# blackfeather-wang/AdaFocus

Measured on AMD Instinct MI355X. Metric: clips/sec (T=16, patch=96^2, ResNet-50 local), higher is better.
Workload: dtype f32; 1 GPU; ActivityNet AdaFocus hot path: gather + ResNet-50 local CNN + GRU classifier, T=16, P=96, B=64 clips/GPU (1024 patches/GPU/step), random-init weights seed 1007; global_batch=64, frames=16, patch=96, parallelism=dp1, streams=3

## Files before the change

### adafocus_amd/csrc/adaf_internal.h

```cpp
#pragma once
#include <hip/hip_runtime.h>
#include <stdint.h>
#include <stddef.h>
#include <string>

#include "../../include/adafocus.h"
#include <type_traits>

struct adaf_handle {
    int device = 0;
    int cus = 256;
    float* zeros = nullptr;
    unsigned* scan_timeouts = nullptr;
    int conv_pos_major = 1;
    int gru_persistent = 1;
    hipEvent_t scan_done[4] = {nullptr, nullptr, nullptr, nullptr};
    bool scan_used[4] = {false, false, false, false};
    int scan_next = 0;
    int scan_resident = 0;
    int scan_slots = 1;
    int bptt_resident = 0;
    std::string err;
};

#include <mutex>
#include <vector>
struct AdafAuxPool {
    struct Aux { hipStream_t key = nullptr; hipStream_t stream = nullptr; hipEvent_t ev_fork = nullptr, ev_join = nullptr; unsigned long long used = 0; };
    static constexpr size_t kMax = 16;
    std::vector<Aux> entries;
    std::mutex mu;
    unsigned long long tick = 0;
    AdafAuxPool() { entries.reserve(kMax); }
    bool create(Aux* a) {
        return hipStreamCreateWithFlags(&a->stream, hipStreamNonBlocking) == hipSuccess &&
               hipEventCreateWithFlags(&a->ev_fork, hipEventDisableTiming) == hipSuccess &&
               hipEventCreateWithFlags(&a->ev_join, hipEventDisableTiming) == hipSuccess;
    }
    void prepare(size_t count) {
        std::lock_guard<std::mutex> lk(mu);
        while (entries.size() < count && entries.size() < kMax) {
            Aux a;
            if (!create(&a)) return;
            entries.push_back(a);
        }
    }
// ... 51 lines not shown
    explicit AdafCarver(void* ws) : base(static_cast<char*>(ws)) {}
    template <typename T> T* take(size_t count, size_t align = sizeof(T)) {
        T* p = base ? reinterpret_cast<T*>(base + off) : nullptr;
        off += (count * sizeof(T) + align - 1) / align * align;
        return p;
    }
};

struct AdafOptions {
    int conv_pool = 1;
    int mb_strip = 1;
    int mbv2_chunk = 512;
    int latency_rows = 1536;
    int latency_linear_rows = 128;
    unsigned effnet_plan = 511u;
    unsigned effnet_fused_blocks = 0xffffffffu;
    int effnet_chunk = 1024;
    int stem_rows = 1;
    int split_stage1_f32 = 1;
    int split_lean = 1;
    int tsm_lean = 1;
    int gru_graph_persistent = 0;
    int gru_scan_slices = 2;
};
AdafOptions& adaf_options();

__device__ __forceinline__ _Float16 adaf_f16_of(float v) {
#if defined(__HIP_DEVICE_COMPILE__)
    asm("" : "+v"(v));
#endif
    return (_Float16)v;
}

struct ConvArgs {
    const float* x;
    const float* w;
    const unsigned short* wsp;
    const float* scale;
    const float* bias;
    const float* res;
    float* out;
    int M, N, K;
    int cin, H, W, OH, OW, KH, KW, stride, pad;
    int ldx, ldo, ldr;
    int act;
    int tsm_T, tsm_fold, tsm_hw;
// ... 122 lines not shown
bool adaf_gru_scan_persistent_ok(int batch, int hidden, int classes, int resident_blocks);
int adaf_gru_scan_groups(int batch, int resident_blocks);
struct AdafGruScanPlan {
    int groups;
    int bpad;
    size_t nzero;
};
AdafGruScanPlan adaf_gru_scan_plan(int batch, int steps, size_t bar_words, int resident_blocks);
hipError_t adaf_launch_gru_scan_persistent(const float* gi, const float* whh, const float* bhh, const float* h0, float* hs,
                                           unsigned* bar, const AdafGruScanPlan& plan, int batch, int steps, const float* fcw, const float* fcb,
                                           float* logits, float* last, int classes, bool cooperative, unsigned* timeouts, hipStream_t s);

int adaf_gru_bptt_blocks_per_cu();
bool adaf_gru_bptt_persistent_ok(int batch, int hidden, int resident_blocks);
hipError_t adaf_launch_gru_bptt(const float* dy, const float* gi, const float* gh, const float* bhh, const float* hs, const float* whh,
                                float* dgi, float* dgh, float* carry, unsigned* bar, unsigned* timeouts, int batch, int steps, int hidden,
                                bool persistent, bool cooperative, hipStream_t s);
void adaf_launch_gemm_strided(const float* A, long long a_m, long long a_k, const float* B, long long b_k, long long b_n, float* C, int ldc,
                              const float* mul, int ldm, int M, int N, int K, hipStream_t s);
size_t adaf_colsum_partial_floats(int cols);
void adaf_launch_colsum(const float* x, int rows, int cols, int ld, float* part, float* out, hipStream_t s);
void adaf_launch_rows_scale(const float* x, const float* mask, float* out, int rows, int width, int steps, bool shift, hipStream_t s);

int adaf_launch_conv_gemm(const ConvArgs& a, int tile, int cus, hipStream_t s);
int adaf_pick_conv_tile(int M, int N, int K, int cus);
int adaf_launch_conv_lat(const ConvArgs& a, hipStream_t s);
int adaf_launch_conv_pool(ConvArgs a, int hw, float* pool_out, int pool_ld, hipStream_t s);
int adaf_launch_conv_pool16(ConvArgs a, int hw, float* pool_out, int pool_ld, hipStream_t s);
int adaf_launch_conv_pool16_rounded(ConvArgs a, int hw, float* pool_out, int pool_ld, hipStream_t s);
bool adaf_conv_tile_exists(int tile);
void adaf_launch_conv_naive(const ConvArgs& a, hipStream_t s);
bool adaf_fused_tail_shift_ok(const ConvArgs& c2, int n3, int ldr, int tsm_T1, int tsm_fold1);
int adaf_launch_fused_tail(const ConvArgs& c2, const float* w3, const float* s3, const float* b3, const float* res, int ldr,
                           float* out, int n3, const float* w1n, const float* s1n, const float* b1n, float* out1, int n1,
                           hipStream_t s, int tsm_T1 = 0, int tsm_fold1 = 0);

hipError_t adaf_launch_crop(const float* frames, int nf, int C, int H, int W, const float* act, int fpa, int P,
                            float* out, int layout, int32_t* coords, hipStream_t s);

hipError_t adaf_launch_crop_resize(const float* frames, int in4, int nf, int C, int H, int W, const float* act, const int32_t* sizes,
                                   int size_default, int fpa, int P, float* out, int layout, int32_t* coords, hipStream_t s);
hipError_t adaf_launch_resize_nearest(const float* frames, int in4, int nf, int C, int H, int W, int OH, int OW, float* out,
                                      int layout, hipStream_t s);

void adaf_launch_split_weight(const float* w, size_t count, unsigned short* planes, hipStream_t s);
void adaf_launch_pack_weight(const float* w, int cout, int cin, int kh, int kw, int cin_pad, float* o, hipStream_t s);
void adaf_launch_fold_bn(const float* g, const float* b, const float* m, const float* v, float eps, int c,
                         float* scale, float* bias, hipStream_t s);
// ... 36 lines not shown
```

### adafocus_amd/csrc/api.hip

```cpp
#include <cstdarg>
#include <cstdio>
#include <cstring>

#include "adaf_internal.h"

int adaf_fail(adaf_handle* h, int code, const char* fmt, ...) {
    char buf[512];
    va_list ap;
    va_start(ap, fmt);
    vsnprintf(buf, sizeof(buf), fmt, ap);
    va_end(ap);
    if (h) h->err = buf;
    return code;
}

int adaf_hip_fail(adaf_handle* h, hipError_t e, const char* what) {
    return adaf_fail(h, ADAF_E_LAUNCH, "%s: %s", what, hipGetErrorString(e));
}

bool adaf_aligned16(const void* p) { return (reinterpret_cast<uintptr_t>(p) & 15) == 0; }
int adaf_check_ws(adaf_handle* h, const char* who, const void* ws, size_t ws_bytes, size_t need, AdafWsOrder order) {
    const bool small = ws_bytes < need, skew = !adaf_aligned16(ws);
    if (small && (order == ADAF_WS_SIZE_FIRST || !skew)) return adaf_fail(h, ADAF_E_NOMEM, "%s: workspace %zu < %zu bytes", who, ws_bytes, need);
    return skew ? adaf_fail(h, ADAF_E_LAYOUT, "%s: the workspace must be 16-byte aligned", who) : ADAF_OK;
// ... 37 lines not shown
    a->vec_epi = (p->cout % 4 == 0 && ldo % 4 == 0 && ldr % 4 == 0 && adaf_aligned16(out) && (!res || adaf_aligned16(res)) &&
                  (!scale || adaf_aligned16(scale)) && (!bias || adaf_aligned16(bias))) ? 1 : 0;
    return ADAF_OK;
}

int adaf_set_conv_dtypes(adaf_handle* h, bool in16, bool out16, ConvArgs* a) {
    a->in16 = in16; a->out16 = out16; a->res16 = a->res != nullptr;
    if (in16 && (a->cin % 8 || a->ldx % 8)) return adaf_fail(h, ADAF_E_LAYOUT, "conv_f16: fp16 operands need cin %% 8 == 0 (16-byte chunks)");
    if (in16 && a->tsm_T > 0 && a->tsm_fold % 8)
        return adaf_fail(h, ADAF_E_LAYOUT, "conv_f16: temporal-shift fold=%d must be a multiple of 8 with fp16 operands (whole 16-byte chunks)", a->tsm_fold);
    if (!in16 && a->res) return adaf_fail(h, ADAF_E_BADARG, "conv_f16: a residual needs fp16 operands");
    return ADAF_OK;
}

AdafOptions& adaf_options() {
    static AdafOptions o;
    return o;
}

namespace {
struct OptKey { const char* name; double lo, hi; };
const OptKey kOptKeys[] = {{"conv_pool", 0, 1}, {"mb_strip", 0, 1}, {"mbv2_chunk", 1, 1 << 20}, {"latency_rows", 0, 1 << 30}, {"latency_linear_rows", 0, 1 << 30},
                           {"effnet_plan", 0, 511}, {"effnet_chunk", 1, 1 << 20}, {"gru_scan_slices", 1, 2}, {"effnet_fused_blocks", 0, 4294967295.0},
                           {"stem_rows", 0, 2}, {"split_stage1_f32", 0, 1}, {"gru_graph_persistent", 0, 1}, {"split_lean", 0, 1}, {"tsm_lean", 0, 1}};
int find_opt(const char* key) {
    if (!key) return -1;
    for (size_t i = 0; i < sizeof(kOptKeys) / sizeof(kOptKeys[0]); ++i)
        if (!strcmp(kOptKeys[i].name, key)) return (int)i;
    return -1;
}
}

extern "C" {

int adaf_version(void) { return ADAF_VERSION; }

int adaf_create(int device, adaf_handle** out) {
    if (!out) return ADAF_E_BADARG;
    *out = nullptr;
    int count = 0;
    if (hipGetDeviceCount(&count) != hipSuccess || device < 0 || device >= count) return ADAF_E_ARCH;
    hipDeviceProp_t prop;
    if (hipGetDeviceProperties(&prop, device) != hipSuccess) return ADAF_E_ARCH;
    if (strncmp(prop.gcnArchName, "gfx950", 6) != 0) return ADAF_E_ARCH;
    adaf_handle* h = new adaf_handle();
    h->device = device;
    h->cus = prop.multiProcessorCount > 0 ? prop.multiProcessorCount : 256;
// ... 5 lines not shown
    if (e == hipSuccess) e = hipMalloc(reinterpret_cast<void**>(&h->scan_timeouts), 256);
    if (e == hipSuccess) e = hipMemset(h->scan_timeouts, 0, 256);
    for (int i = 0; i < 4 && e == hipSuccess; ++i) e = hipEventCreateWithFlags(&h->scan_done[i], hipEventDisableTiming);
    if (e == hipSuccess) {
        const int per_cu = adaf_gru_scan_blocks_per_cu();
        h->scan_resident = (per_cu > 1 ? per_cu - 1 : per_cu) * h->cus;
        const int slots = h->scan_resident / 128;
        h->scan_slots = slots < 1 ? 1 : (slots > 4 ? 4 : slots);
        const int bptt_per_cu = adaf_gru_bptt_blocks_per_cu();
        h->bptt_resident = (bptt_per_cu > 1 ? bptt_per_cu - 1 : bptt_per_cu) * h->cus;
    }
    (void)hipSetDevice(cur);
    if (e != hipSuccess) { delete h; return ADAF_E_NOMEM; }
    *out = h;
    return ADAF_OK;
}

int adaf_destroy(adaf_handle* h) {
    if (h && h->zeros) (void)hipFree(h->zeros);
    if (h && h->scan_timeouts) (void)hipFree(h->scan_timeouts);
    if (h)
        for (int i = 0; i < 4; ++i)
            if (h->scan_done[i]) (void)hipEventDestroy(h->scan_done[i]);
    delete h;
    return ADAF_OK;
}

const char* adaf_last_error(const adaf_handle* h) { return h ? h->err.c_str() : "null handle"; }
int adaf_device_cus(const adaf_handle* h) { return h ? h->cus : 0; }
int adaf_set_conv_pos_major(adaf_handle* h, int on) {
    if (!h) return ADAF_E_BADARG;
    h->conv_pos_major = on < 0 || on > 2 ? 1 : on;
    return ADAF_OK;
}
int adaf_set_global_option(const char* key, double value) {
    const int k = find_opt(key);
    if (k < 0 || !(value >= kOptKeys[k].lo && value <= kOptKeys[k].hi)) return ADAF_E_BADARG;
    AdafOptions& o = adaf_options();
    switch (k) {
        case 0: o.conv_pool = (int)value; break;
        case 1: o.mb_strip = (int)value; break;
        case 2: o.mbv2_chunk = (int)value; break;
        case 3: o.latency_rows = (int)value; break;
        case 4: o.latency_linear_rows = (int)value; break;
        case 5: o.effnet_plan = (unsigned)value; break;
        case 6: o.effnet_chunk = (int)value; break;
        case 7: o.gru_scan_slices = (int)value; break;
        case 8: o.effnet_fused_blocks = (unsigned)value; break;
        case 9: o.stem_rows = (int)value; break;
        case 10: o.split_stage1_f32 = (int)value; break;
        case 11: o.gru_graph_persistent = (int)value; break;
        case 12: o.split_lean = (int)value; break;
        default: o.tsm_lean = (int)value; break;
    }
    return ADAF_OK;
}

double adaf_get_global_option(const char* key) {
    const AdafOptions& o = adaf_options();
    switch (find_opt(key)) {
        case 0: return o.conv_pool;
        case 1: return o.mb_strip;
        case 2: return o.mbv2_chunk;
        case 3: return o.latency_rows;
        case 4: return o.latency_linear_rows;
        case 5: return o.effnet_plan;
        case 6: return o.effnet_chunk;
        case 7: return o.gru_scan_slices;
        case 8: return o.effnet_fused_blocks;
        case 9: return o.stem_rows;
        case 10: return o.split_stage1_f32;
        case 11: return o.gru_graph_persistent;
        case 12: return o.split_lean;
        case 13: return o.tsm_lean;
        default: return __builtin_nan("");
    }
}

int adaf_set_gru_persistent(adaf_handle* h, int on) {
    if (!h) return ADAF_E_BADARG;
    if (on < 0 || on > 2) return adaf_fail(h, ADAF_E_BADARG, "set_gru_persistent: mode %d (0 off, 1 on, 2 on + cooperative launch)", on);
    h->gru_persistent = on;
    return ADAF_OK;
}

int adaf_gru_scan_timeouts(adaf_handle* h, unsigned* count_out) {
    if (!h || !count_out) return ADAF_E_BADARG;
    int cur = 0;
    (void)hipGetDevice(&cur);
    (void)hipSetDevice(h->device);
    hipError_t e = hipDeviceSynchronize();
    if (e == hipSuccess) e = hipMemcpy(count_out, h->scan_timeouts, sizeof(unsigned), hipMemcpyDeviceToHost);
    (void)hipSetDevice(cur);
    return e == hipSuccess ? ADAF_OK : adaf_hip_fail(h, e, "gru_scan_timeouts");
}

int adaf_crop_gather_f32(adaf_handle* h, const float* frames, int n_frames, int channels, int height, int width,
// ... 520 lines not shown
```

### adafocus_amd/csrc/conv_gemm.hip

```cpp
#include <cstdlib>
#include <type_traits>
#include <utility>

#include "adaf_internal.h"

typedef float f32x16 __attribute__((ext_vector_type(16)));
typedef float f32x4 __attribute__((ext_vector_type(4)));
typedef float f32x2 __attribute__((ext_vector_type(2)));
typedef unsigned u32x4 __attribute__((ext_vector_type(4)));
typedef __bf16 bf16x8 __attribute__((ext_vector_type(8)));
typedef _Float16 f16x8 __attribute__((ext_vector_type(8)));
typedef _Float16 f16x4 __attribute__((ext_vector_type(4)));

#ifndef CG_ABL
#define CG_ABL 0
#endif

namespace {

typedef __bf16 bf16x2 __attribute__((ext_vector_type(2)));
__device__ __forceinline__ void split3(const f32x4 v0, const f32x4 v1, u32x4& H, u32x4& M, u32x4& L) {
    const float x[8] = {v0.x, v0.y, v0.z, v0.w, v1.x, v1.y, v1.z, v1.w};
    unsigned h[4], m[4], l[4];
#pragma unroll
// ... 1447 lines not shown
    else if (a.act == ADAF_ACT_SWISH) v = v / (1.f + expf(-v));
    a.out[(size_t)m * a.ldo + n] = v;
}

enum TileFamily {
    TF_REG,
    TF_DMA_TOP,
    TF_DMA_MID,
    TF_BAR23,
    TF_SPLIT6,
    TF_SPLIT9,
    TF_PRESPLIT,
    TF_F16,
    TF_LAT,
};
struct TileRow {
    int id;
    int bm, bn;
    int wgm, wgn;
    TileFamily fam;
    int fallback;
    int presplit;
    float eff;
};
constexpr int kTileAutoSplit = 40;
constexpr TileRow kTileTable[] = {
    {1, 128, 128, 2, 2, TF_REG, 0, 0, 1.00f},
    {2, 128, 64, 2, 2, TF_REG, 0, 0, 1.02f},
    {3, 64, 64, 2, 2, TF_REG, 0, 0, 0.98f},
    {4, 64, 128, 2, 2, TF_REG, 0, 0, 0.99f},
    {5, 256, 128, 4, 2, TF_REG, 0, 0, 0.f},
    {21, 128, 128, 2, 2, TF_DMA_TOP, 1, 0, 0.f},
    {22, 128, 64, 2, 2, TF_DMA_TOP, 2, 0, 0.f},
    {23, 64, 64, 2, 2, TF_DMA_TOP, 3, 0, 0.f},
    {24, 64, 128, 2, 2, TF_DMA_TOP, 4, 0, 0.f},
    {25, 256, 128, 4, 2, TF_DMA_TOP, 5, 0, 0.f},
    {26, 256, 128, 2, 2, TF_DMA_TOP, 1, 0, 0.f},
    {31, 128, 128, 2, 2, TF_DMA_MID, 1, 0, 0.f},
    {32, 128, 64, 2, 2, TF_DMA_MID, 2, 0, 0.f},
    {33, 64, 64, 2, 2, TF_DMA_MID, 3, 0, 0.f},
    {34, 64, 128, 2, 2, TF_DMA_MID, 4, 0, 0.f},
    {38, 128, 32, 4, 1, TF_DMA_MID, 1, 0, 0.f},
    {39, 256, 32, 4, 1, TF_DMA_MID, 1, 0, 0.f},
    {41, 128, 128, 2, 2, TF_SPLIT6, 1, 65, 0.f},
    {42, 128, 64, 2, 2, TF_SPLIT6, 2, 62, 0.f},
    {43, 64, 64, 2, 2, TF_SPLIT6, 3, 63, 0.f},
    {44, 64, 128, 2, 2, TF_SPLIT6, 4, 64, 0.f},
    {45, 256, 128, 4, 2, TF_SPLIT6, 5, 0, 0.f},
    {46, 256, 128, 2, 2, TF_SPLIT6, 1, 0, 0.f},
    {51, 128, 128, 2, 2, TF_SPLIT9, 1, 0, 0.f},
    {52, 128, 64, 2, 2, TF_SPLIT9, 2, 0, 0.f},
    {53, 64, 64, 2, 2, TF_SPLIT9, 3, 0, 0.f},
    {54, 64, 128, 2, 2, TF_SPLIT9, 4, 0, 0.f},
// ... 63 lines not shown
};

bool conv_is_dense(const ConvArgs& a) { return a.KH == 1 && a.KW == 1 && a.stride == 1 && a.pad == 0; }
int conv_images(const ConvArgs& a) { return a.OH * a.OW > 0 ? a.M / (a.OH * a.OW) : 0; }

bool dma_reach(size_t elems, size_t elem_bytes = 4) { return elems * elem_bytes < 0xffffff00ull; }
bool operands_in_dma_reach(const ConvArgs& a) {
    return dma_reach((size_t)a.M * a.ldx) && dma_reach((size_t)a.N * a.K) &&
           (conv_is_dense(a) || dma_reach((size_t)a.H * a.W * a.ldx * (size_t)conv_images(a)));
}
bool strided_1x1_as_gather(const ConvArgs& a) {
    return !conv_is_dense(a) && a.KH == 1 && a.KW == 1 && a.pad == 0 && a.stride > 1 && a.tsm_T == 0 && (a.K & 31) == 0;
}

double conv_tap_fill(const ConvArgs& a) {
    auto axis = [&](int out, int in, int k) {
        long long c = 0;
        for (int o = 0; o < out; ++o)
            for (int t = 0; t < k; ++t) c += (unsigned)(o * a.stride - a.pad + t) < (unsigned)in;
        return c;
    };
    return (double)(axis(a.OH, a.H, a.KH) * axis(a.OW, a.W, a.KW)) / ((double)a.OH * a.OW * a.KH * a.KW);
}
bool pos_major_gate(const ConvArgs& a, const TileRow& r) {
    const int ohw = a.OH * a.OW, images = conv_images(a);
    return has_pos_major_form(r) && (r.fam == TF_PRESPLIT ? a.pm_allow == 1 : a.pm_allow != 0) && !conv_is_dense(a) && a.KH * a.KW > 1 &&
           a.KH * a.KW <= 32 && images * ohw == a.M && images >= r.bm && ohw <= 4096 && conv_tap_fill(a) < 0.96;
}
bool lean_shift_gate(const ConvArgs& a, const TileRow& r) {
    return has_lean_shift_form(r) && conv_is_dense(a) && a.tsm_T > 0 && (a.K & 31) == 0 && (a.tsm_fold & 31) == 0 && a.stride == 1 &&
           operands_in_dma_reach(a) && adaf_options().tsm_lean && (size_t)a.M * a.ldx * 4 < 0x7fff0000ull;
}

bool adaf_conv_glds_ok(const ConvArgs& a) {
    if (conv_is_dense(a)) return a.K % 4 == 0;
    return a.K % 32 == 0 && a.cin % 32 == 0 && a.KH * a.KW <= 32;
}

bool conv_glds16_ok(const ConvArgs& a) {
    if ((a.K & 1) || (a.cin & 1) || (a.ldx & 1)) return false;
    if (conv_is_dense(a)) return (a.K / 2) % 4 == 0;
    return (a.K / 2) % 32 == 0 && (a.cin / 2) % 32 == 0 && a.KH * a.KW <= 32;
}

bool narrow_output(const ConvArgs& a) { return (((a.N + 63) / 64) * 64 - a.N) * 5 >= a.N; }
long long row_tiles(const ConvArgs& a, int bm) { return (a.M + bm - 1) / bm; }

int resolve_f32_tile(const ConvArgs& a, int tile, int cus) {
    const bool dma_ok = adaf_conv_glds_ok(a);
    const bool presplit_ok = a.wsp != nullptr && (a.K & 31) == 0 && dma_ok;
    if (tile == kTileAutoSplit) {
        tile = 0;
        if (dma_ok) {
            if (a.N <= 64) tile = family_tile(TF_SPLIT6, 128, 64);
            else if (row_tiles(a, 128) * ((a.N + 127) / 128) * 2 >= cus) tile = family_tile(TF_SPLIT6, 128, 128);
            else tile = family_tile_like(TF_SPLIT6, adaf_pick_conv_tile(a.M, a.N, a.K, cus));
            if (presplit_ok) tile = kTileTable[tile_index(tile)].presplit;
        }
    }
    if (tile <= 0) {
        tile = adaf_pick_conv_tile(a.M, a.N, a.K, cus);
        if (dma_ok) {
            tile = family_tile_like(TF_DMA_MID, tile);
            if (narrow_output(a) && row_tiles(a, 128) >= cus) tile = family_tile(TF_DMA_MID, 128, 32);
            else if (narrow_output(a) && a.K >= 512 && row_tiles(a, 256) * ((a.N + 31) / 32) >= cus) tile = family_tile(TF_DMA_MID, 256, 32);
        }
    }
    for (int i = tile_index(tile); i >= 0; i = tile_index(tile)) {
        const TileRow& r = kTileTable[i];
        if (r.fam == TF_REG || (r.fam == TF_PRESPLIT ? presplit_ok : dma_ok && r.fam != TF_F16 && r.fam != TF_LAT)) return tile;
        tile = r.fallback;
    }
    return -1;
}

void plan_row_major(ConvPlan& p, const ConvArgs& a, int tile, int bm_rows) {
    p.row = tile_index(p.tile = tile);
    p.a.tiles_n = (a.N + kTileTable[p.row].bn - 1) / kTileTable[p.row].bn;
    p.a.nblocks = ((a.M + bm_rows - 1) / bm_rows) * p.a.tiles_n;
}

ConvPlan plan_conv(const ConvArgs& a, int tile, int cus) {
    ConvPlan p(a);
    const bool dense = conv_is_dense(a);
    if (a.in16) {
        if (!conv_glds16_ok(a) || (a.res && !a.res16)) return p;
        if (tile < kTileF16Lo || tile > kTileF16Hi) {
            tile = family_tile_like(TF_F16, adaf_pick_conv_tile(a.M, a.N, a.K, cus));
            if (narrow_output(a) && row_tiles(a, 128) >= cus) tile = family_tile(TF_F16, 128, 32);
        }
        if (tile_index(tile) < 0) return p;
        plan_row_major(p, a, tile, kTileTable[tile_index(tile)].bm);
        p.a.K /= 2; p.a.cin /= 2; p.a.ldx /= 2; p.a.tsm_fold /= 2;
        p.dt = DT_IN16 | DT_RES16 | (a.out16 ? DT_OUT16 : 0);
        p.dense = dense;
        p.special = dense && (a.tsm_T > 0 || (p.a.K & 31));
        return p;
    }
    if (a.out16) {
        if (a.res) return p;
        plan_row_major(p, a, kTileOut16, kTileTable[tile_index(kTileOut16)].bm);
        p.dt = DT_OUT16;
        p.dense = dense;
        return p;
    }
    const int asked = tile_index(tile);
    if (asked >= 0 && kTileTable[asked].fam == TF_LAT) {
        p.row = tile_index(p.tile = tile);
        return p;
    }
    tile = resolve_f32_tile(a, tile, cus);
    if (tile < 0) return p;
    const TileRow& r = kTileTable[tile_index(tile)];
    plan_row_major(p, a, tile, r.bm);
    if (a.vec_epi) p.a.vec_epi = 2;
    p.dense = dense;
    if (r.fam == TF_REG) return p;
    const bool special = a.tsm_T > 0 || (a.K & 31);
    p.special = dense && special;
    const bool lean = has_lean_form(r) && operands_in_dma_reach(a) &&
                      (r.fam != TF_PRESPLIT || (adaf_options().split_lean && dma_reach((size_t)3 * a.N * a.K, 2)));
    if (pos_major_gate(a, r)) {
        p.pos_major = true;
        p.lean = lean && a.pm_allow != 2;
        p.a.pm_images = conv_images(a);
        p.a.pm_groups = (p.a.pm_images + r.bm - 1) / r.bm;
        p.a.nblocks = a.OH * a.OW * p.a.pm_groups * p.a.tiles_n;
    } else if ((dense || strided_1x1_as_gather(a)) && !special && lean && lean_dense_pays(r)) {
        p.gather = !dense;
        p.dense = p.lean = true;
    } else if (lean_shift_gate(a, r)) {
        p.lean = true;
    }
    return p;
// ... 70 lines not shown
}

template <int... I>
int launch_rows(const ConvPlan& p, const ConvArgs& a, hipStream_t s, std::integer_sequence<int, I...>) {
    int rc = -1;
    (void)((p.row == I && ((rc = launch_row<I>(p, a, s)), true)) || ...);
    return rc;
}

int launch_plan(const ConvPlan& p, hipStream_t s) {
    return p.tile < 0 ? -1 : launch_rows(p, p.a, s, std::make_integer_sequence<int, kNumTiles>());
}

int launch_conv_pool(const ConvArgs& a, int hw, float* pool_out, int pool_ld, PoolKind kind, hipStream_t s) {
    ConvPlan p = plan_conv_pool(a, hw, pool_out, pool_ld, kind);
    if (p.tile < 0) return 0;
    p.a.pool_hw = hw; p.a.pool_rows = (128 / hw) * hw; p.a.pool_out = pool_out; p.a.pool_ld = pool_ld;
    launch_plan(p, s);
    return 1;
}

}

int adaf_pick_conv_tile(int M, int N, int K, int cus) {
    (void)K;
    int best = 1;
    double best_t = 1e300;
    for (const TileRow& r : kTileTable) {
        if (r.eff <= 0.f) continue;
        const long long blocks = (long long)((M + r.bm - 1) / r.bm) * ((N + r.bn - 1) / r.bn);
        const long long rounds = (blocks + cus - 1) / cus;
        const double cost = (double)rounds * r.bm * r.bn / r.eff;
        if (cost < best_t * 0.999) { best_t = cost; best = r.id; }
    }
    return best;
}

bool adaf_conv_tile_exists(int tile) { return tile == kTileAutoSplit || tile_index(tile) >= 0; }

int adaf_launch_conv_gemm(const ConvArgs& a, int tile, int cus, hipStream_t s) { return launch_plan(plan_conv(a, tile, cus), s); }

int adaf_launch_conv_pool(ConvArgs a, int hw, float* pool_out, int pool_ld, hipStream_t s) {
    return launch_conv_pool(a, hw, pool_out, pool_ld, POOL_F32, s);
}

int adaf_launch_conv_pool16(ConvArgs a, int hw, float* pool_out, int pool_ld, hipStream_t s) {
    return launch_conv_pool(a, hw, pool_out, pool_ld, POOL_F16, s);
}

int adaf_launch_conv_pool16_rounded(ConvArgs a, int hw, float* pool_out, int pool_ld, hipStream_t s) {
    return launch_conv_pool(a, hw, pool_out, pool_ld, POOL_F16_ROUNDED, s);
}

extern "C" int adaf_conv_plan_debug(const adaf_conv_params* p, int flags, int cus, int* out, int n) {
    enum { IN16 = 1, OUT16 = 2, RES16 = 4, PRESPLIT = 8, VEC_EPI = 64 };
    alignas(16) static const float operand[4] = {0.f, 0.f, 0.f, 0.f};
    alignas(16) static float result[4];
    if (!out || cus <= 0) return ADAF_E_BADARG;
    adaf_handle host;
    ConvArgs a;
    int rc = adaf_make_conv_args(&host, p, operand, operand, nullptr, nullptr, (flags & RES16) ? operand : nullptr, result, &a);
    if (!rc && (flags & (IN16 | OUT16 | RES16))) rc = adaf_set_conv_dtypes(&host, (flags & IN16) != 0, (flags & OUT16) != 0, &a);
    if (rc) return rc;
    if (flags & PRESPLIT) a.wsp = reinterpret_cast<const unsigned short*>(operand);
    a.pm_allow = (flags >> 4) & 3;
    a.vec_epi = a.vec_epi && (flags & VEC_EPI);
    const int hw = flags >> 8;
    const ConvPlan c = hw > 0 ? plan_conv_pool(a, hw, operand, p->cout, !a.in16 ? POOL_F32 : a.res16 ? POOL_F16_ROUNDED : POOL_F16)
                              : plan_conv(a, p->tile, cus);
    const TileRow r = c.row >= 0 ? kTileTable[c.row] : TileRow{0, 0, 0, 0, 0, TF_REG, 0, 0, 0.f};
    const int kPlanFields[] = {c.tile, r.bm, r.bn, r.wgm, r.wgn, (int)r.fam, r.fallback, family_pipe(r.fam), family_split(r.fam),
                               r.fam == TF_PRESPLIT, c.dt, c.dense, c.gather, c.special, c.lean, c.pos_major, c.pool, c.a.tiles_n, c.a.nblocks,
                               c.a.pm_images, c.a.pm_groups, c.a.vec_epi, c.a.K, c.a.cin, c.a.ldx, c.a.tsm_fold};
    for (int i = 0; i < n && i < (int)(sizeof(kPlanFields) / sizeof(int)); ++i) out[i] = kPlanFields[i];
    return ADAF_OK;
}

void adaf_launch_conv_naive(const ConvArgs& a, hipStream_t s) {
    const long long total = (long long)a.M * a.N;
    hipLaunchKernelGGL(conv_naive_kernel, dim3((unsigned)((total + 255) / 256)), dim3(256), 0, s, a);
}

static bool fused_tail_pm(const ConvArgs& c2, int n3, int ldr, int* images_out, int* groups_out, int gstride = 128) {
    const int ohw = c2.OH * c2.OW;
    const int images = ohw > 0 ? c2.M / ohw : 0;
    const int groups = (images + gstride - 1) / gstride;
    *images_out = images;
    *groups_out = groups;
    return c2.pm_allow == 1 && images * ohw == c2.M && images >= 128 && ohw <= 4096 &&
           (long long)groups * 128 * 100 <= (long long)images * (gstride == 128 ? 106 : 108) && (size_t)ohw * 8 * (size_t)(n3 > ldr ? n3 : ldr) * 4 < 0xffffff00ull;
}

static int fused_tail_gstride(int tsm_T1) { return tsm_T1 > 0 && tsm_T1 <= 128 ? (128 / tsm_T1) * tsm_T1 : 128; }
// ... 48 lines not shown
```

### adafocus_amd/csrc/resnet_trunk.hip

```cpp
#include <cstdio>
#include <cstring>
#include <string>
#include <vector>

#include "adaf_net.h"

struct ConvLayer : AdafNetConv {
    int pad;
    bool tsm = false;
    unsigned short* wsp = nullptr;
};

struct adaf_resnet50 {
    adaf_handle* h = nullptr;
    AdafParamTable params;
    AdafWeightArena arena;
    std::vector<ConvLayer> convs;
    std::vector<int> tiles;
    int blocks[4] = {3, 4, 6, 3};
    float* l10_w = nullptr;
    float* l10_scale = nullptr;
    float* l10_bias = nullptr;
    unsigned short* l10_w16 = nullptr;
    int math = ADAF_MATH_F32;
// ... 48 lines not shown
    int nframes, H, W;
    const float* act;
    int fpa;
};

adaf_conv_params layer_params(const ConvLayer& L, int n, int hh, int ww, int act) {
    adaf_conv_params p;
    memset(&p, 0, sizeof(p));
    p.n = n; p.h = hh; p.w = ww; p.cin = L.cin_pad; p.cout = L.cout; p.kh = p.kw = L.k; p.stride = L.stride; p.pad = L.pad;
    p.act = act;
    return p;
}

size_t trunk_layout(const adaf_resnet50* net, int n, int patch, void* ws, float* buf[6]) {
    const int s1 = adaf_conv_out(patch, 7, 2, 3), s2 = adaf_conv_out(s1, 3, 2, 1);
    const size_t a = (size_t)s1 * s1 * 64, b = (size_t)s2 * s2 * 256;
    AdafCarver c(ws);
    for (int i = 0; i < 6; ++i) buf[i] = (i < 5 || (net && net->tsm_block)) ? c.take<float>((a > b ? a : b) * n) : nullptr;
    return c.off;
}

inline const float* as_f32(const void* p) { return static_cast<const float*>(p); }

int run_trunk(adaf_resnet50* net, const float* x4, int n, int P, int tsm_T, int tsm_div, float* feat, int ldfeat,
              void* ws, size_t ws_bytes, hipStream_t st, std::vector<hipEvent_t>* rec, std::vector<Launch>* info, float* featmap = nullptr,
              const FrameSrc* src = nullptr) {
    adaf_handle* h = net->h;
    if (src) x4 = src->frames;
    if (!net->finalized) return adaf_fail(h, ADAF_E_STATE, "resnet50: finalize() has not been called");
    if (!x4 || !feat || !ws) return adaf_fail(h, ADAF_E_BADARG, "resnet50: null pointer");
    if (n <= 0 || P < 32) return adaf_fail(h, ADAF_E_BADARG, "resnet50: need n > 0 and patch >= 32");
    if (ldfeat == 0) ldfeat = 2048;
    if (ldfeat < 2048 || ldfeat % 4 || !adaf_aligned16(feat) || !adaf_aligned16(x4) || !adaf_aligned16(ws))
        return adaf_fail(h, ADAF_E_LAYOUT, "resnet50: ldfeat >= 2048, %% 4 == 0 and 16-byte aligned buffers required");
    if (tsm_T > 0 && n % tsm_T) return adaf_fail(h, ADAF_E_BADARG, "resnet50: n=%d not a multiple of tsm_segments=%d", n, tsm_T);
    float* buf[6];
    if (int rc = adaf_check_ws(h, "resnet50", ws, ws_bytes, trunk_layout(net, n, P, ws, buf), ADAF_WS_ALIGN_FIRST)) return rc;

    const int lat_rows = net->lat_rows >= 0 ? net->lat_rows : adaf_options().latency_rows;
    const bool lat_ok = lat_rows > 0 && tsm_T == 0 && net->math == ADAF_MATH_F32;
    const bool fuse = net->fuse;
    const bool stage1_f32 = net->math == ADAF_MATH_F32 || (net->math == ADAF_MATH_F32_SPLIT_BF16 && adaf_options().split_stage1_f32);
    const bool tsm_block = net->tsm_block && tsm_T > 0;
    const int tsm_c1 = tsm_block ? 0 : tsm_T;

    const bool f16 = net->math == ADAF_MATH_F16;
    const double eb = f16 ? 2.0 : 4.0;
    const char* tag = f16 ? " (fp16)" : "";
    if (f16) {
        if (!net->convs[1].w16) return adaf_fail(h, ADAF_E_STATE, "resnet50: fp16 filters missing (finalize() did not complete)");
        if (tsm_T > 0 && tsm_div <= 0) return adaf_fail(h, ADAF_E_BADARG, "resnet50: tsm_div must be positive");
        if (tsm_c1 > 0)
            for (size_t i = 1; i < net->convs.size(); ++i) {
                const ConvLayer& L = net->convs[i];
                if (L.tsm && (L.cin / tsm_div) % 8)
                    return adaf_fail(h, ADAF_E_LAYOUT, "resnet50 (fp16): temporal-shift fold = %d / %d = %d of %s must be a multiple of 8", L.cin, tsm_div,
                                     L.cin / tsm_div, L.name.c_str());
            }
    }
    auto bank = [&](const ConvLayer& L) { return f16 ? as_f32(L.w16) : L.w; };
    const float* const l10_w = f16 ? as_f32(net->l10_w16) : (stage1_f32 ? net->l10_w : nullptr);

    auto mark = [&](double flops, double bytes, int tile) {
        if (rec) {
            (void)hipEventRecord((*rec)[info->size()], st);
            info->push_back({flops, bytes, tile});
        }
    };
    int li = 0;
    bool pooled = false;
    auto conv = [&](const float* in, int hh, int ww, int act, const float* res, float* out, bool tsm, int* oh, int* ow) -> int {
        const ConvLayer& L = net->convs[li];
        adaf_conv_params p = layer_params(L, n, hh, ww, act);
        p.tsm_segments = tsm ? tsm_T : 0; p.tsm_div = tsm_div;
        const bool split_here = net->math == ADAF_MATH_F32_SPLIT_BF16 && !(stage1_f32 && li >= 1 && li <= 11);
        p.tile = net->tiles[li] ? net->tiles[li] : (split_here ? 40 : 0);
        ConvArgs a;
        int rc = adaf_make_conv_args(h, &p, in, bank(L), L.scale, L.bias, res, out, &a);
        if (rc) return rc;
        a.wsp = split_here ? L.wsp : nullptr;
        if (f16) { a.in16 = a.out16 = 1; a.res16 = res != nullptr; }
        const double macs = (double)a.M * L.cout * L.k * L.k * L.cin;
        const double bytes = eb * ((double)n * hh * ww * L.cin + (double)a.M * L.cout * (res ? 2 : 1) + (double)L.cout * L.k * L.k * L.cin);
        mark(2.0 * macs, bytes, 0);
        const bool want_lat = lat_ok && a.M <= lat_rows && li > 0 && !net->tiles[li];
        int used = adaf_launch_conv_gemm(a, want_lat ? 95 : p.tile, h->cus, st);
        if (used < 0 && want_lat) used = adaf_launch_conv_gemm(a, p.tile, h->cus, st);
        if (used < 0) return adaf_fail(h, ADAF_E_LAUNCH, "resnet50%s: no kernel for tile id %d (conv launch %d)", tag, p.tile, li);
        if (info && !info->empty()) info->back().tile = used;
        *oh = a.OH; *ow = a.OW;
        ++li;
        return ADAF_OK;
    };

    const ConvLayer& L0 = net->convs[0];
    const int s1 = adaf_conv_out(P, 7, 2, 3), ph = adaf_conv_out(s1, 3, 2, 1);
    const double stem_flops = 2.0 * (double)n * s1 * s1 * 64 * 147;
    const double stem_in = 4.0 * ((double)n * P * P * 3 + 64.0 * 147), conv_map = 4.0 * (double)n * s1 * s1 * 64, pool_map = eb * (double)n * ph * ph * 64;
    const bool stem_kernel = net->tiles[0] == 0;
    int rc;
    bool gathered = false;
    if (src) {
        if (stem_kernel && fuse && adaf_stem7x7_rows_ok(P, n, h->cus)) {
            mark(stem_flops, stem_in + pool_map, 94);
            gathered = adaf_launch_stem7x7_pool_frames(src->frames, src->pixel_major, src->nframes, src->act, src->fpa, src->H, src->W, n, P,
                                                       net->stem_w, L0.scale, L0.bias, buf[1], h->cus, st, f16);
            if (!gathered && rec) info->pop_back();
        }
        if (!gathered) {
            mark(0.0, 4.0 * 2.0 * (double)n * P * P * 3, 0);
// ... 142 lines not shown
int adaf_resnet50_create(adaf_handle* h, adaf_resnet50** out) {
    if (!h || !out) return ADAF_E_BADARG;
    adaf_resnet50* net = new adaf_resnet50();
    net->h = h;
    build_layers(net);
    *out = net;
    return ADAF_OK;
}

int adaf_resnet50_destroy(adaf_resnet50* net) {
    if (!net) return ADAF_OK;
    net->arena.release();
    delete net;
    return ADAF_OK;
}

int adaf_resnet50_set_param(adaf_resnet50* net, const char* name, const float* dev_ptr, size_t numel) {
    if (!net || !name || !dev_ptr) return ADAF_E_BADARG;
    net->params.set(name, dev_ptr, numel);
    net->finalized = false;
    return ADAF_OK;
}

static int split_weights(adaf_resnet50* net, void* stream) {
    adaf_handle* h = net->h;
    hipStream_t st = (hipStream_t)stream;
    for (size_t i = 1; i < net->convs.size(); ++i) {
        ConvLayer& L = net->convs[i];
        const size_t wn = L.packed_floats();
        if (!net->arena.take(&L.wsp, 3 * wn))
            return adaf_fail(h, ADAF_E_NOMEM, "resnet50: hipMalloc split weights");
        adaf_launch_split_weight(L.w, wn, L.wsp, st);
    }
    hipError_t e = hipStreamSynchronize(st);
    if (e != hipSuccess) return adaf_hip_fail(h, e, "resnet50 split weights");
    return ADAF_OK;
}

static int f16_weights(adaf_resnet50* net, void* stream) {
    adaf_handle* h = net->h;
    hipStream_t st = (hipStream_t)stream;
    for (size_t i = 1; i < net->convs.size(); ++i) {
        ConvLayer& L = net->convs[i];
        const size_t wn = L.packed_floats();
        if (!net->arena.take(&L.w16, wn))
            return adaf_fail(h, ADAF_E_NOMEM, "resnet50: hipMalloc fp16 weights");
// ... 200 lines not shown
```

Before: 5450 clips/s.

## Pick conv tiles with a busy-device cost model when other streams run trunks

Tracks, per handle, an event recorded after each ResNet trunk forward on each stream. At the start of a trunk it checks whether another stream's forward is still in flight. If so, f32 conv tile selection switches to a 'busy' cost model that assumes the neighbour streams fill part of the tail wave and uses lower per-tile efficiencies. It also groups pos-major convs by image. This aims to avoid tiles sized for an idle GPU when three streams share the CUs, at the cost of an event query per forward and a host-timing-dependent tile choice.

```diff
diff --git a/adafocus_amd/csrc/adaf_internal.h b/adafocus_amd/csrc/adaf_internal.h
--- a/adafocus_amd/csrc/adaf_internal.h
+++ b/adafocus_amd/csrc/adaf_internal.h
@@ -3,6 +3,7 @@
 #include <stdint.h>
 #include <stddef.h>
 #include <string>
+#include <mutex>
 
 #include "../../include/adafocus.h"
 #include <type_traits>
@@ -20,8 +21,16 @@
     int scan_resident = 0;
     int scan_slots = 1;
     int bptt_resident = 0;
+    static constexpr int kWatched = 8;
+    hipStream_t watch_key[kWatched] = {};
+    hipEvent_t watch_done[kWatched] = {};
+    unsigned long long watch_used[kWatched] = {};
+    unsigned long long watch_tick = 0;
+    std::mutex watch_mu;
     std::string err;
 };
+bool adaf_launches_beside(adaf_handle* h, hipStream_t st);
+void adaf_note_forward(adaf_handle* h, hipStream_t st);
 
 #include <mutex>
 #include <vector>
@@ -119,6 +128,7 @@
     int tsm_lean = 1;
     int gru_graph_persistent = 0;
     int gru_scan_slices = 2;
+    int conv_tile_regime = 1;
 };
 AdafOptions& adaf_options();
 
@@ -287,8 +297,7 @@
 void adaf_launch_colsum(const float* x, int rows, int cols, int ld, float* part, float* out, hipStream_t s);
 void adaf_launch_rows_scale(const float* x, const float* mask, float* out, int rows, int width, int steps, bool shift, hipStream_t s);
 
-int adaf_launch_conv_gemm(const ConvArgs& a, int tile, int cus, hipStream_t s);
-int adaf_pick_conv_tile(int M, int N, int K, int cus);
+int adaf_launch_conv_gemm(const ConvArgs& a, int tile, int cus, hipStream_t s, bool beside = false);
 int adaf_launch_conv_lat(const ConvArgs& a, hipStream_t s);
 int adaf_launch_conv_pool(ConvArgs a, int hw, float* pool_out, int pool_ld, hipStream_t s);
 int adaf_launch_conv_pool16(ConvArgs a, int hw, float* pool_out, int pool_ld, hipStream_t s);
diff --git a/adafocus_amd/csrc/api.hip b/adafocus_amd/csrc/api.hip
--- a/adafocus_amd/csrc/api.hip
+++ b/adafocus_amd/csrc/api.hip
@@ -83,7 +83,7 @@
 struct OptKey { const char* name; double lo, hi; };
 const OptKey kOptKeys[] = {{"conv_pool", 0, 1}, {"mb_strip", 0, 1}, {"mbv2_chunk", 1, 1 << 20}, {"latency_rows", 0, 1 << 30}, {"latency_linear_rows", 0, 1 << 30},
                            {"effnet_plan", 0, 511}, {"effnet_chunk", 1, 1 << 20}, {"gru_scan_slices", 1, 2}, {"effnet_fused_blocks", 0, 4294967295.0},
-                           {"stem_rows", 0, 2}, {"split_stage1_f32", 0, 1}, {"gru_graph_persistent", 0, 1}, {"split_lean", 0, 1}, {"tsm_lean", 0, 1}};
+                           {"stem_rows", 0, 2}, {"split_stage1_f32", 0, 1}, {"gru_graph_persistent", 0, 1}, {"split_lean", 0, 1}, {"tsm_lean", 0, 1}, {"conv_tile_regime", 0, 2}};
 int find_opt(const char* key) {
     if (!key) return -1;
     for (size_t i = 0; i < sizeof(kOptKeys) / sizeof(kOptKeys[0]); ++i)
@@ -135,9 +135,46 @@
     if (h)
         for (int i = 0; i < 4; ++i)
             if (h->scan_done[i]) (void)hipEventDestroy(h->scan_done[i]);
+    if (h)
+        for (int i = 0; i < adaf_handle::kWatched; ++i)
+            if (h->watch_done[i]) (void)hipEventDestroy(h->watch_done[i]);
     delete h;
     return ADAF_OK;
 }
+
+}
+
+namespace {
+bool stream_capturing(hipStream_t st) {
+    hipStreamCaptureStatus cap = hipStreamCaptureStatusNone;
+    (void)hipStreamIsCapturing(st, &cap);
+    return cap != hipStreamCaptureStatusNone;
+}
+}
+
+bool adaf_launches_beside(adaf_handle* h, hipStream_t st) {
+    if (!h || stream_capturing(st)) return false;
+    std::lock_guard<std::mutex> lock(h->watch_mu);
+    for (int i = 0; i < adaf_handle::kWatched; ++i)
+        if (h->watch_done[i] && h->watch_used[i] && h->watch_key[i] != st && hipEventQuery(h->watch_done[i]) == hipErrorNotReady) return true;
+    return false;
+}
+
+void adaf_note_forward(adaf_handle* h, hipStream_t st) {
+    if (!h || stream_capturing(st)) return;
+    std::lock_guard<std::mutex> lock(h->watch_mu);
+    int slot = 0;
+    for (int i = 0; i < adaf_handle::kWatched; ++i) {
+        if (h->watch_used[i] && h->watch_key[i] == st) { slot = i; break; }
+        if (h->watch_used[i] < h->watch_used[slot]) slot = i;
+    }
+    if (!h->watch_done[slot] && hipEventCreateWithFlags(&h->watch_done[slot], hipEventDisableTiming) != hipSuccess) { h->watch_done[slot] = nullptr; return; }
+    h->watch_key[slot] = st;
+    h->watch_used[slot] = ++h->watch_tick;
+    (void)hipEventRecord(h->watch_done[slot], st);
+}
+
+extern "C" {
 
 const char* adaf_last_error(const adaf_handle* h) { return h ? h->err.c_str() : "null handle"; }
 int adaf_device_cus(const adaf_handle* h) { return h ? h->cus : 0; }
@@ -164,7 +201,8 @@
         case 10: o.split_stage1_f32 = (int)value; break;
         case 11: o.gru_graph_persistent = (int)value; break;
         case 12: o.split_lean = (int)value; break;
-        default: o.tsm_lean = (int)value; break;
+        case 13: o.tsm_lean = (int)value; break;
+        default: o.conv_tile_regime = (int)value; break;
     }
     return ADAF_OK;
 }
@@ -186,6 +224,7 @@
         case 11: return o.gru_graph_persistent;
         case 12: return o.split_lean;
         case 13: return o.tsm_lean;
+        case 14: return o.conv_tile_regime;
         default: return __builtin_nan("");
     }
 }
diff --git a/adafocus_amd/csrc/conv_gemm.hip b/adafocus_amd/csrc/conv_gemm.hip
--- a/adafocus_amd/csrc/conv_gemm.hip
+++ b/adafocus_amd/csrc/conv_gemm.hip
@@ -1493,13 +1493,14 @@
     int fallback;
     int presplit;
     float eff;
+    float eff_busy;
 };
 constexpr int kTileAutoSplit = 40;
 constexpr TileRow kTileTable[] = {
-    {1, 128, 128, 2, 2, TF_REG, 0, 0, 1.00f},
-    {2, 128, 64, 2, 2, TF_REG, 0, 0, 1.02f},
-    {3, 64, 64, 2, 2, TF_REG, 0, 0, 0.98f},
-    {4, 64, 128, 2, 2, TF_REG, 0, 0, 0.99f},
+    {1, 128, 128, 2, 2, TF_REG, 0, 0, 1.00f, 0.80f},
+    {2, 128, 64, 2, 2, TF_REG, 0, 0, 1.02f, 0.82f},
+    {3, 64, 64, 2, 2, TF_REG, 0, 0, 0.98f, 0.76f},
+    {4, 64, 128, 2, 2, TF_REG, 0, 0, 0.99f, 0.79f},
     {5, 256, 128, 4, 2, TF_REG, 0, 0, 0.f},
     {21, 128, 128, 2, 2, TF_DMA_TOP, 1, 0, 0.f},
     {22, 128, 64, 2, 2, TF_DMA_TOP, 2, 0, 0.f},
@@ -1609,10 +1610,12 @@
     };
     return (double)(axis(a.OH, a.H, a.KH) * axis(a.OW, a.W, a.KW)) / ((double)a.OH * a.OW * a.KH * a.KW);
 }
+bool pos_major_conv(const ConvArgs& a) {
+    const int ohw = a.OH * a.OW;
+    return !conv_is_dense(a) && a.KH * a.KW > 1 && a.KH * a.KW <= 32 && conv_images(a) * ohw == a.M && ohw <= 4096 && conv_tap_fill(a) < 0.96;
+}
 bool pos_major_gate(const ConvArgs& a, const TileRow& r) {
-    const int ohw = a.OH * a.OW, images = conv_images(a);
-    return has_pos_major_form(r) && (r.fam == TF_PRESPLIT ? a.pm_allow == 1 : a.pm_allow != 0) && !conv_is_dense(a) && a.KH * a.KW > 1 &&
-           a.KH * a.KW <= 32 && images * ohw == a.M && images >= r.bm && ohw <= 4096 && conv_tap_fill(a) < 0.96;
+    return has_pos_major_form(r) && (r.fam == TF_PRESPLIT ? a.pm_allow == 1 : a.pm_allow != 0) && pos_major_conv(a) && conv_images(a) >= r.bm;
 }
 bool lean_shift_gate(const ConvArgs& a, const TileRow& r) {
     return has_lean_shift_form(r) && conv_is_dense(a) && a.tsm_T > 0 && (a.K & 31) == 0 && (a.tsm_fold & 31) == 0 && a.stride == 1 &&
@@ -1630,10 +1633,31 @@
     return (a.K / 2) % 32 == 0 && (a.cin / 2) % 32 == 0 && a.KH * a.KW <= 32;
 }
 
+constexpr double kNeighbourFill = 0.75;
+
+double conv_tile_cost(long long M, int N, int K, const TileRow& r, int cus, bool busy, int groups = 1) {
+    (void)K;
+    const long long blocks = (long long)groups * ((M + r.bm - 1) / r.bm) * ((N + r.bn - 1) / r.bn);
+    const double fill = busy ? kNeighbourFill : 0.0;
+    const double per_cu = fill * (double)blocks / cus + (1.0 - fill) * (double)((blocks + cus - 1) / cus);
+    return per_cu * r.bm * r.bn / (busy ? r.eff_busy : r.eff);
+}
+int pick_tile(long long M, int N, int K, int cus, bool busy, int groups = 1, long long group_rows = 0) {
+    int best = 1;
+    double best_t = 1e300;
+    for (const TileRow& r : kTileTable) {
+        if (r.eff <= 0.f) continue;
+        const bool grouped = groups > 1 && group_rows >= r.bm;
+        const double cost = grouped ? conv_tile_cost(group_rows, N, K, r, cus, busy, groups) : conv_tile_cost(M, N, K, r, cus, busy);
+        if (cost < best_t * 0.999) { best_t = cost; best = r.id; }
+    }
+    return best;
+}
+
 bool narrow_output(const ConvArgs& a) { return (((a.N + 63) / 64) * 64 - a.N) * 5 >= a.N; }
 long long row_tiles(const ConvArgs& a, int bm) { return (a.M + bm - 1) / bm; }
 
-int resolve_f32_tile(const ConvArgs& a, int tile, int cus) {
+int resolve_f32_tile(const ConvArgs& a, int tile, int cus, bool beside) {
     const bool dma_ok = adaf_conv_glds_ok(a);
     const bool presplit_ok = a.wsp != nullptr && (a.K & 31) == 0 && dma_ok;
     if (tile == kTileAutoSplit) {
@@ -1641,12 +1665,15 @@
         if (dma_ok) {
             if (a.N <= 64) tile = family_tile(TF_SPLIT6, 128, 64);
             else if (row_tiles(a, 128) * ((a.N + 127) / 128) * 2 >= cus) tile = family_tile(TF_SPLIT6, 128, 128);
-            else tile = family_tile_like(TF_SPLIT6, adaf_pick_conv_tile(a.M, a.N, a.K, cus));
+            else tile = family_tile_like(TF_SPLIT6, pick_tile(a.M, a.N, a.K, cus, false));
             if (presplit_ok) tile = kTileTable[tile_index(tile)].presplit;
         }
     }
     if (tile <= 0) {
-        tile = adaf_pick_conv_tile(a.M, a.N, a.K, cus);
+        const int regime = adaf_options().conv_tile_regime;
+        const bool busy = (regime == 2 || (regime == 1 && beside)) && dma_ok;
+        const bool pm = busy && a.pm_allow != 0 && pos_major_conv(a);
+        tile = pm ? pick_tile(a.M, a.N, a.K, cus, busy, a.OH * a.OW, conv_images(a)) : pick_tile(a.M, a.N, a.K, cus, busy);
         if (dma_ok) {
             tile = family_tile_like(TF_DMA_MID, tile);
             if (narrow_output(a) && row_tiles(a, 128) >= cus) tile = family_tile(TF_DMA_MID, 128, 32);
@@ -1667,13 +1694,13 @@
     p.a.nblocks = ((a.M + bm_rows - 1) / bm_rows) * p.a.tiles_n;
 }
 
-ConvPlan plan_conv(const ConvArgs& a, int tile, int cus) {
+ConvPlan plan_conv(const ConvArgs& a, int tile, int cus, bool beside = false) {
     ConvPlan p(a);
     const bool dense = conv_is_dense(a);
     if (a.in16) {
         if (!conv_glds16_ok(a) || (a.res && !a.res16)) return p;
         if (tile < kTileF16Lo || tile > kTileF16Hi) {
-            tile = family_tile_like(TF_F16, adaf_pick_conv_tile(a.M, a.N, a.K, cus));
+            tile = family_tile_like(TF_F16, pick_tile(a.M, a.N, a.K, cus, false));
             if (narrow_output(a) && row_tiles(a, 128) >= cus) tile = family_tile(TF_F16, 128, 32);
         }
         if (tile_index(tile) < 0) return p;
@@ -1696,7 +1723,7 @@
         p.row = tile_index(p.tile = tile);
         return p;
     }
-    tile = resolve_f32_tile(a, tile, cus);
+    tile = resolve_f32_tile(a, tile, cus, beside);
     if (tile < 0) return p;
     const TileRow& r = kTileTable[tile_index(tile)];
     plan_row_major(p, a, tile, r.bm);
@@ -1813,23 +1840,9 @@
 
 }
 
-int adaf_pick_conv_tile(int M, int N, int K, int cus) {
-    (void)K;
-    int best = 1;
-    double best_t = 1e300;
-    for (const TileRow& r : kTileTable) {
-        if (r.eff <= 0.f) continue;
-        const long long blocks = (long long)((M + r.bm - 1) / r.bm) * ((N + r.bn - 1) / r.bn);
-        const long long rounds = (blocks + cus - 1) / cus;
-        const double cost = (double)rounds * r.bm * r.bn / r.eff;
-        if (cost < best_t * 0.999) { best_t = cost; best = r.id; }
-    }
-    return best;
-}
-
 bool adaf_conv_tile_exists(int tile) { return tile == kTileAutoSplit || tile_index(tile) >= 0; }
 
-int adaf_launch_conv_gemm(const ConvArgs& a, int tile, int cus, hipStream_t s) { return launch_plan(plan_conv(a, tile, cus), s); }
+int adaf_launch_conv_gemm(const ConvArgs& a, int tile, int cus, hipStream_t s, bool beside) { return launch_plan(plan_conv(a, tile, cus, beside), s); }
 
 int adaf_launch_conv_pool(ConvArgs a, int hw, float* pool_out, int pool_ld, hipStream_t s) {
     return launch_conv_pool(a, hw, pool_out, pool_ld, POOL_F32, s);
@@ -1844,7 +1857,7 @@
 }
 
 extern "C" int adaf_conv_plan_debug(const adaf_conv_params* p, int flags, int cus, int* out, int n) {
-    enum { IN16 = 1, OUT16 = 2, RES16 = 4, PRESPLIT = 8, VEC_EPI = 64 };
+    enum { IN16 = 1, OUT16 = 2, RES16 = 4, PRESPLIT = 8, VEC_EPI = 64, BESIDE = 128 };
     alignas(16) static const float operand[4] = {0.f, 0.f, 0.f, 0.f};
     alignas(16) static float result[4];
     if (!out || cus <= 0) return ADAF_E_BADARG;
@@ -1858,8 +1871,8 @@
     a.vec_epi = a.vec_epi && (flags & VEC_EPI);
     const int hw = flags >> 8;
     const ConvPlan c = hw > 0 ? plan_conv_pool(a, hw, operand, p->cout, !a.in16 ? POOL_F32 : a.res16 ? POOL_F16_ROUNDED : POOL_F16)
-                              : plan_conv(a, p->tile, cus);
-    const TileRow r = c.row >= 0 ? kTileTable[c.row] : TileRow{0, 0, 0, 0, 0, TF_REG, 0, 0, 0.f};
+                              : plan_conv(a, p->tile, cus, (flags & BESIDE) != 0);
+    const TileRow r = c.row >= 0 ? kTileTable[c.row] : TileRow{0, 0, 0, 0, 0, TF_REG, 0, 0, 0.f, 0.f};
     const int kPlanFields[] = {c.tile, r.bm, r.bn, r.wgm, r.wgn, (int)r.fam, r.fallback, family_pipe(r.fam), family_split(r.fam),
                                r.fam == TF_PRESPLIT, c.dt, c.dense, c.gather, c.special, c.lean, c.pos_major, c.pool, c.a.tiles_n, c.a.nblocks,
                                c.a.pm_images, c.a.pm_groups, c.a.vec_epi, c.a.K, c.a.cin, c.a.ldx, c.a.tsm_fold};
diff --git a/adafocus_amd/csrc/resnet_trunk.hip b/adafocus_amd/csrc/resnet_trunk.hip
--- a/adafocus_amd/csrc/resnet_trunk.hip
+++ b/adafocus_amd/csrc/resnet_trunk.hip
@@ -94,9 +94,9 @@
 
 inline const float* as_f32(const void* p) { return static_cast<const float*>(p); }
 
-int run_trunk(adaf_resnet50* net, const float* x4, int n, int P, int tsm_T, int tsm_div, float* feat, int ldfeat,
-              void* ws, size_t ws_bytes, hipStream_t st, std::vector<hipEvent_t>* rec, std::vector<Launch>* info, float* featmap = nullptr,
-              const FrameSrc* src = nullptr) {
+int walk_trunk(adaf_resnet50* net, const float* x4, int n, int P, int tsm_T, int tsm_div, float* feat, int ldfeat,
+               void* ws, size_t ws_bytes, hipStream_t st, std::vector<hipEvent_t>* rec, std::vector<Launch>* info, float* featmap,
+               const FrameSrc* src) {
     adaf_handle* h = net->h;
     if (src) x4 = src->frames;
     if (!net->finalized) return adaf_fail(h, ADAF_E_STATE, "resnet50: finalize() has not been called");
@@ -112,6 +112,7 @@
     const int lat_rows = net->lat_rows >= 0 ? net->lat_rows : adaf_options().latency_rows;
     const bool lat_ok = lat_rows > 0 && tsm_T == 0 && net->math == ADAF_MATH_F32;
     const bool fuse = net->fuse;
+    const bool beside = adaf_launches_beside(h, st);
     const bool stage1_f32 = net->math == ADAF_MATH_F32 || (net->math == ADAF_MATH_F32_SPLIT_BF16 && adaf_options().split_stage1_f32);
     const bool tsm_block = net->tsm_block && tsm_T > 0;
     const int tsm_c1 = tsm_block ? 0 : tsm_T;
@@ -156,8 +157,8 @@
         const double bytes = eb * ((double)n * hh * ww * L.cin + (double)a.M * L.cout * (res ? 2 : 1) + (double)L.cout * L.k * L.k * L.cin);
         mark(2.0 * macs, bytes, 0);
         const bool want_lat = lat_ok && a.M <= lat_rows && li > 0 && !net->tiles[li];
-        int used = adaf_launch_conv_gemm(a, want_lat ? 95 : p.tile, h->cus, st);
-        if (used < 0 && want_lat) used = adaf_launch_conv_gemm(a, p.tile, h->cus, st);
+        int used = adaf_launch_conv_gemm(a, want_lat ? 95 : p.tile, h->cus, st, beside);
+        if (used < 0 && want_lat) used = adaf_launch_conv_gemm(a, p.tile, h->cus, st, beside);
         if (used < 0) return adaf_fail(h, ADAF_E_LAUNCH, "resnet50%s: no kernel for tile id %d (conv launch %d)", tag, p.tile, li);
         if (info && !info->empty()) info->back().tile = used;
         *oh = a.OH; *ow = a.OW;
@@ -346,6 +347,14 @@
     return ADAF_OK;
 }
 
+static int run_trunk(adaf_resnet50* net, const float* x4, int n, int P, int tsm_T, int tsm_div, float* feat, int ldfeat,
+              void* ws, size_t ws_bytes, hipStream_t st, std::vector<hipEvent_t>* rec, std::vector<Launch>* info, float* featmap = nullptr,
+              const FrameSrc* src = nullptr) {
+    const int rc = walk_trunk(net, x4, n, P, tsm_T, tsm_div, feat, ldfeat, ws, ws_bytes, st, rec, info, featmap, src);
+    if (rc == ADAF_OK) adaf_note_forward(net->h, st);
+    return rc;
+}
+
 static int split_weights(adaf_resnet50* net, void* stream) {
     adaf_handle* h = net->h;
     hipStream_t st = (hipStream_t)stream;
```

Result: faster. 5537 clips/s (median of 6 runs) (+1.6%).
